# espnet/espnet

Measured on NVIDIA B200. Metric: utterances/sec (RTF) Conformer-large ASR inference at 1/2/4/8 B200 vs CPU ref, higher is better.
Workload: dtype f32

## Files before the change

espnet_b200/csrc/gemm.cu:

```cuda
#include <cuda.h>
#include <limits.h>
#include <stdio.h>
#include <stdlib.h>

#include "common.cuh"
#include "gemm.h"
#include "tc_common.cuh"

namespace {

using namespace espb::tc;

constexpr int BM = 128;
constexpr int BK = 32;
constexpr int A_TILE_BYTES = BM * 128;
constexpr int NUM_THREADS = 192;

struct EpiArgs {
  float* C; long long c_plane, ldc; int split_out;
  const float* bias; const float* R; long long ldr; float alpha; int act;
};

__device__ __forceinline__ float epi_value(const EpiArgs& e, float acc, long long row, int col) {
  float v = acc;
// ... 3 lines not shown
  if (e.R) v += e.R[row * e.ldr + col];
  return v;
}

__device__ __forceinline__ void epi_store_chunk32(const EpiArgs& e, float (&v)[32], int row, bool row_ok, int col0, int N, bool vec_ok, bool r_vec_ok) {
  float* crow = e.C + (long long)row * e.ldc;
  if (!row_ok || col0 >= N) return;
  if (vec_ok && col0 + 32 <= N) {
    float rres[32];
    if (e.R && r_vec_ok) {
      const float4* rp4 = reinterpret_cast<const float4*>(e.R + (long long)row * e.ldr + col0);
#pragma unroll
      for (int j = 0; j < 8; ++j) { const float4 t = rp4[j]; rres[4 * j] = t.x; rres[4 * j + 1] = t.y; rres[4 * j + 2] = t.z; rres[4 * j + 3] = t.w; }
    } else {
#pragma unroll
      for (int j = 0; j < 32; ++j) rres[j] = e.R ? e.R[(long long)row * e.ldr + col0 + j] : 0.f;
    }
#pragma unroll
    for (int j = 0; j < 32; ++j) {
      float x = v[j];
      if (e.bias) x += __ldg(e.bias + col0 + j);
      x = espb::apply_act_acc(x, e.act);
      v[j] = fmaf(e.alpha, x, rres[j]);
    }
#pragma unroll
    for (int j = 0; j < 32; j += 4) {
      float4 o, l;
      const float t0 = v[j], t1 = v[j + 1], t2 = v[j + 2], t3 = v[j + 3];
      if (e.split_out) {
        o.x = espb::tf32_hi(t0); o.y = espb::tf32_hi(t1); o.z = espb::tf32_hi(t2); o.w = espb::tf32_hi(t3);
        l.x = espb::tf32_lo(t0, o.x); l.y = espb::tf32_lo(t1, o.y); l.z = espb::tf32_lo(t2, o.z); l.w = espb::tf32_lo(t3, o.w);
        *reinterpret_cast<float4*>(crow + col0 + j) = o;
        *reinterpret_cast<float4*>(crow + e.c_plane + col0 + j) = l;
      } else {
        o.x = t0; o.y = t1; o.z = t2; o.w = t3;
        *reinterpret_cast<float4*>(crow + col0 + j) = o;
      }
    }
  } else {
#pragma unroll
    for (int j = 0; j < 32; ++j) {
      const int col = col0 + j;
      if (col < N) {
        const float t = epi_value(e, v[j], row, col);
        if (e.split_out) {
          const float h = espb::tf32_hi(t);
          crow[col] = h; crow[e.c_plane + col] = espb::tf32_lo(t, h);
        } else {
          crow[col] = t;
        }
      }
    }
  }
}

template <int BN, int STAGES>
__global__ void __launch_bounds__(NUM_THREADS, 1)
gemm_tf32x3_kernel(const __grid_constant__ CUtensorMap tmA, const __grid_constant__ CUtensorMap tmB, EspbGemmDesc p, int bxm, int bym, int axm, int aym) {
  constexpr int B_TILE_BYTES = BN * 128;
  constexpr int STAGE_BYTES = 2 * A_TILE_BYTES + 2 * B_TILE_BYTES;
  extern __shared__ uint8_t smem_raw[];
  const uint32_t smem_base = (smem_u32(smem_raw) + 1023u) & ~1023u;
  const uint32_t bar_base = smem_base + STAGES * STAGE_BYTES;
  const uint32_t full_bar = bar_base, empty_bar = bar_base + 8 * STAGES, tmem_full_bar = bar_base + 16 * STAGES;
  uint32_t* tmem_ptr_smem = reinterpret_cast<uint32_t*>(smem_raw + (bar_base - smem_u32(smem_raw)) + 16 * STAGES + 8);

  const int warp = threadIdx.x >> 5, lane = threadIdx.x & 31;
  const int m0 = blockIdx.x * BM, n0 = blockIdx.y * BN;
  const int bx = blockIdx.z % p.nbx, by = blockIdx.z / p.nbx;
  const int num_kb = (p.K + BK - 1) / BK;
  if (p.band_t > 0 && ((n0 + BN - 1 < p.band_t - 1 - (m0 + BM - 1)) || (n0 > 2 * p.band_t - 2 - m0))) {
    espb::pdl_wait();
    return;
  }

  if (warp == 0 && lane == 0) {
    for (int s = 0; s < STAGES; ++s) { mbar_init(full_bar + 8 * s, 1); mbar_init(empty_bar + 8 * s, 1); }
    mbar_init(tmem_full_bar, 1);
    asm volatile("fence.mbarrier_init.release.cluster;" ::: "memory");
    asm volatile("prefetch.tensormap [%0];" ::"l"(&tmA) : "memory");
    asm volatile("prefetch.tensormap [%0];" ::"l"(&tmB) : "memory");
  }
  if (warp == 1) {
    asm volatile("tcgen05.alloc.cta_group::1.sync.aligned.shared::cta.b32 [%0], %1;" ::"r"(smem_u32(tmem_ptr_smem)), "r"((uint32_t)BN) : "memory");
    asm volatile("tcgen05.relinquish_alloc_permit.cta_group::1.sync.aligned;" ::: "memory");
  }
  tcgen05_fence_before();
  __syncthreads();
  tcgen05_fence_after();
  const uint32_t tmem_base = *tmem_ptr_smem;
  espb::pdl_trigger();
  espb::pdl_wait();

  if (warp == 0) {
    if (elect_one_sync()) {
      const int cblk = (p.a_mode == 1) ? p.cv_cin / BK : 0;
      for (int kb = 0; kb < num_kb; ++kb) {
        const int s = kb % STAGES;
        const uint32_t ph = (kb / STAGES) & 1;
        mbar_wait(empty_bar + 8 * s, ph ^ 1);
        const uint32_t fb = full_bar + 8 * s;
        mbar_expect_tx(fb, STAGE_BYTES);
        const uint32_t sa = smem_base + s * STAGE_BYTES;
        if (p.a_mode == 0) {
          const int ko = (p.kob > 0) ? kb / p.kob : 0;
          const int ki = (p.kob > 0) ? kb % p.kob : kb;
// ... 48 lines not shown
    const bool r_vec_ok = p.R && ((p.ldr & 3) == 0) && ((((long long)by * p.sr_y + (long long)bx * p.sr_x) & 3) == 0) &&
                          ((reinterpret_cast<uintptr_t>(p.R) & 15) == 0);
#pragma unroll 1
    for (int c = 0; c < BN / 32; ++c) {
      float v[32];
      __syncwarp();
      tmem_ld32(tmem_base + ((uint32_t)(q * 32) << 16) + (uint32_t)(c * 32), v);
      epi_store_chunk32(e, v, row, row_ok, n0 + c * 32, p.N, vec_ok, r_vec_ok);
    }
  }
  tcgen05_fence_before();
  __syncthreads();
  if (warp == 1) {
    asm volatile("tcgen05.dealloc.cta_group::1.sync.aligned.b32 %0, %1;" ::"r"(tmem_base), "r"((uint32_t)BN) : "memory");
  }
}

template <int BN, int STAGES, int MC>
__global__ void __cluster_dims__(1, MC, 1) __launch_bounds__(NUM_THREADS, 1)
gemm_tf32x3_mc_kernel(const __grid_constant__ CUtensorMap tmA, const __grid_constant__ CUtensorMap tmB, EspbGemmDesc p, int bxm, int bym, int axm, int aym) {
  constexpr int B_TILE_BYTES = BN * 128;
  constexpr int STAGE_BYTES = 2 * A_TILE_BYTES + 2 * B_TILE_BYTES;
  extern __shared__ uint8_t smem_raw[];
  const uint32_t smem_base = (smem_u32(smem_raw) + 1023u) & ~1023u;
  const uint32_t bar_base = smem_base + STAGES * STAGE_BYTES;
  const uint32_t full_bar = bar_base, empty_bar = bar_base + 8 * STAGES, tmem_full_bar = bar_base + 16 * STAGES;
  uint32_t* tmem_ptr_smem = reinterpret_cast<uint32_t*>(smem_raw + (bar_base - smem_u32(smem_raw)) + 16 * STAGES + 8);

  const int warp = threadIdx.x >> 5, lane = threadIdx.x & 31;
  const int m0 = blockIdx.x * BM, n0 = blockIdx.y * BN;
  const int bx = blockIdx.z % p.nbx, by = blockIdx.z / p.nbx;
  const int num_kb = (p.K + BK - 1) / BK;
  const uint32_t rank = cluster_ctarank_v();
  constexpr uint16_t MASK = (uint16_t)((1u << MC) - 1);
  constexpr int SLICE_ROWS = BM / MC, SLICE_BYTES = SLICE_ROWS * 128;

  if (warp == 0 && lane == 0) {
    for (int s = 0; s < STAGES; ++s) { mbar_init(full_bar + 8 * s, 1); mbar_init(empty_bar + 8 * s, MC); }
    mbar_init(tmem_full_bar, 1);
    asm volatile("fence.mbarrier_init.release.cluster;" ::: "memory");
    asm volatile("prefetch.tensormap [%0];" ::"l"(&tmA) : "memory");
    asm volatile("prefetch.tensormap [%0];" ::"l"(&tmB) : "memory");
  }
  if (warp == 1) {
    asm volatile("tcgen05.alloc.cta_group::1.sync.aligned.shared::cta.b32 [%0], %1;" ::"r"(smem_u32(tmem_ptr_smem)), "r"((uint32_t)BN) : "memory");
    asm volatile("tcgen05.relinquish_alloc_permit.cta_group::1.sync.aligned;" ::: "memory");
  }
  tcgen05_fence_before();
  __syncthreads();
  cluster_sync_all_v();
  tcgen05_fence_after();
  const uint32_t tmem_base = *tmem_ptr_smem;
  espb::pdl_trigger();
  espb::pdl_wait();

  if (warp == 0) {
    if (elect_one_sync()) {
      for (int kb = 0; kb < num_kb; ++kb) {
        const int s = kb % STAGES;
        const uint32_t ph = (kb / STAGES) & 1;
        mbar_wait(empty_bar + 8 * s, ph ^ 1);
        const uint32_t fb = full_bar + 8 * s;
        mbar_expect_tx(fb, STAGE_BYTES);
        const uint32_t sa = smem_base + s * STAGE_BYTES;
        {
          const int ko = (p.kob > 0) ? kb / p.kob : 0;
          const int ki = (p.kob > 0) ? kb % p.kob : kb;
          const int mrow = m0 + (int)rank * SLICE_ROWS;
          tma_load_5d_mc(sa + rank * SLICE_BYTES, &tmA, fb, ki * BK, mrow, bx * axm + ko, by * aym, 0, MASK);
          tma_load_5d_mc(sa + A_TILE_BYTES + rank * SLICE_BYTES, &tmA, fb, ki * BK, mrow, bx * axm + ko, by * aym, 1, MASK);
        }
        tma_load_5d(sa + 2 * A_TILE_BYTES, &tmB, fb, kb * BK, n0, bx * bxm, by * bym, 0);
        tma_load_5d(sa + 2 * A_TILE_BYTES + B_TILE_BYTES, &tmB, fb, kb * BK, n0, bx * bxm, by * bym, 1);
      }
    }
  } else if (warp == 1) {
    if (elect_one_sync()) {
      const uint32_t idesc = (1u << 4) | (2u << 7) | (2u << 10) | ((uint32_t)(BN >> 3) << 17) | ((uint32_t)(BM >> 4) << 24);
      for (int kb = 0; kb < num_kb; ++kb) {
        const int s = kb % STAGES;
        const uint32_t ph = (kb / STAGES) & 1;
        mbar_wait(full_bar + 8 * s, ph);
        tcgen05_fence_after();
        const uint32_t sa = smem_base + s * STAGE_BYTES;
#pragma unroll
        for (int k = 0; k < BK / 8; ++k) {
          const uint64_t a_hi = umma_desc(sa + k * 32), a_lo = umma_desc(sa + A_TILE_BYTES + k * 32);
          const uint64_t b_hi = umma_desc(sa + 2 * A_TILE_BYTES + k * 32);
          const uint64_t b_lo = umma_desc(sa + 2 * A_TILE_BYTES + B_TILE_BYTES + k * 32);
          mma_tf32(tmem_base, a_lo, b_hi, idesc, (kb | k) != 0);
          mma_tf32(tmem_base, a_hi, b_lo, idesc, 1);
          mma_tf32(tmem_base, a_hi, b_hi, idesc, 1);
        }
        tcgen05_commit_mc(empty_bar + 8 * s, MASK);
      }
      tcgen05_commit(tmem_full_bar);
    }
  } else {
    const int q = warp & 3;
    mbar_wait(tmem_full_bar, 0);
    tcgen05_fence_after();
    const int row = m0 + q * 32 + lane;
    const bool row_ok = row < p.M;
    EpiArgs e;
    const long long coff = (long long)by * p.sc_y + (long long)bx * p.sc_x;
    e.C = p.C + coff; e.c_plane = p.c_plane; e.ldc = p.ldc; e.split_out = p.split_out;
    e.bias = p.bias ? p.bias + (long long)bx * p.sbias_x : nullptr; e.R = p.R ? p.R + (long long)by * p.sr_y + (long long)bx * p.sr_x : nullptr;
    e.ldr = p.ldr; e.alpha = p.alpha; e.act = p.act;
    const bool vec_ok = ((p.ldc & 3) == 0) && ((coff & 3) == 0) && ((p.c_plane & 3) == 0) &&
                        ((reinterpret_cast<uintptr_t>(p.C) & 15) == 0);
    const bool r_vec_ok = p.R && ((p.ldr & 3) == 0) && ((((long long)by * p.sr_y + (long long)bx * p.sr_x) & 3) == 0) &&
                          ((reinterpret_cast<uintptr_t>(p.R) & 15) == 0);
#pragma unroll 1
    for (int c = 0; c < BN / 32; ++c) {
      float v[32];
      __syncwarp();
      tmem_ld32(tmem_base + ((uint32_t)(q * 32) << 16) + (uint32_t)(c * 32), v);
      epi_store_chunk32(e, v, row, row_ok, n0 + c * 32, p.N, vec_ok, r_vec_ok);
    }
  }
  tcgen05_fence_before();
  __syncthreads();
  cluster_sync_all_v();
  if (warp == 1) {
    asm volatile("tcgen05.dealloc.cta_group::1.sync.aligned.b32 %0, %1;" ::"r"(tmem_base), "r"((uint32_t)BN) : "memory");
  }
}

template <int BN, int STAGES, int SK>
__global__ void __cluster_dims__(1, 1, SK) __launch_bounds__(NUM_THREADS, 1)
gemm_tf32x3_sk_kernel(const __grid_constant__ CUtensorMap tmA, const __grid_constant__ CUtensorMap tmB, EspbGemmDesc p) {
  constexpr int B_TILE_BYTES = BN * 128;
  constexpr int STAGE_BYTES = 2 * A_TILE_BYTES + 2 * B_TILE_BYTES;
  constexpr int NCHUNK = BN / 32;
  static_assert(STAGES * STAGE_BYTES >= BN * BM * 4, "partial-tile staging must fit in the pipeline buffers");
  extern __shared__ uint8_t smem_raw[];
  const uint32_t smem_base = (smem_u32(smem_raw) + 1023u) & ~1023u;
  const uint32_t bar_base = smem_base + STAGES * STAGE_BYTES;
  const uint32_t full_bar = bar_base, empty_bar = bar_base + 8 * STAGES, tmem_full_bar = bar_base + 16 * STAGES;
  uint32_t* tmem_ptr_smem = reinterpret_cast<uint32_t*>(smem_raw + (bar_base - smem_u32(smem_raw)) + 16 * STAGES + 8);

  const int warp = threadIdx.x >> 5, lane = threadIdx.x & 31;
  const int m0 = blockIdx.x * BM, n0 = blockIdx.y * BN;
  const uint32_t rank = cluster_ctarank_v();
  const int num_kb_all = (p.K + BK - 1) / BK;
  const int kb_per = (num_kb_all + SK - 1) / SK;
  const int kb0 = (int)rank * kb_per;
  const int nkb = min(num_kb_all, kb0 + kb_per) - kb0;

  if (warp == 0 && lane == 0) {
    for (int s = 0; s < STAGES; ++s) { mbar_init(full_bar + 8 * s, 1); mbar_init(empty_bar + 8 * s, 1); }
    mbar_init(tmem_full_bar, 1);
    asm volatile("fence.mbarrier_init.release.cluster;" ::: "memory");
    asm volatile("prefetch.tensormap [%0];" ::"l"(&tmA) : "memory");
    asm volatile("prefetch.tensormap [%0];" ::"l"(&tmB) : "memory");
  }
  if (warp == 1) {
    asm volatile("tcgen05.alloc.cta_group::1.sync.aligned.shared::cta.b32 [%0], %1;" ::"r"(smem_u32(tmem_ptr_smem)), "r"((uint32_t)BN) : "memory");
    asm volatile("tcgen05.relinquish_alloc_permit.cta_group::1.sync.aligned;" ::: "memory");
  }
  tcgen05_fence_before();
  __syncthreads();
  tcgen05_fence_after();
  const uint32_t tmem_base = *tmem_ptr_smem;
  espb::pdl_trigger();
  espb::pdl_wait();
  const int q = warp & 3;
  const uint32_t stg_lane = smem_base + (uint32_t)(q * 32 + lane) * 16u;

  if (warp == 0) {
    if (elect_one_sync()) {
      for (int i = 0; i < nkb; ++i) {
        const int s = i % STAGES;
        const uint32_t ph = (i / STAGES) & 1;
        mbar_wait(empty_bar + 8 * s, ph ^ 1);
        const uint32_t fb = full_bar + 8 * s;
        mbar_expect_tx(fb, STAGE_BYTES);
        const uint32_t sa = smem_base + s * STAGE_BYTES;
        const int k0 = (kb0 + i) * BK;
        tma_load_5d(sa, &tmA, fb, k0, m0, 0, 0, 0);
        tma_load_5d(sa + A_TILE_BYTES, &tmA, fb, k0, m0, 0, 0, 1);
        tma_load_5d(sa + 2 * A_TILE_BYTES, &tmB, fb, k0, n0, 0, 0, 0);
        tma_load_5d(sa + 2 * A_TILE_BYTES + B_TILE_BYTES, &tmB, fb, k0, n0, 0, 0, 1);
      }
    }
  } else if (warp == 1) {
    if (elect_one_sync()) {
      const uint32_t idesc = (1u << 4) | (2u << 7) | (2u << 10) | ((uint32_t)(BN >> 3) << 17) | ((uint32_t)(BM >> 4) << 24);
      for (int i = 0; i < nkb; ++i) {
        const int s = i % STAGES;
        const uint32_t ph = (i / STAGES) & 1;
        mbar_wait(full_bar + 8 * s, ph);
        tcgen05_fence_after();
        const uint32_t sa = smem_base + s * STAGE_BYTES;
#pragma unroll
        for (int k = 0; k < BK / 8; ++k) {
          const uint64_t a_hi = umma_desc(sa + k * 32), a_lo = umma_desc(sa + A_TILE_BYTES + k * 32);
          const uint64_t b_hi = umma_desc(sa + 2 * A_TILE_BYTES + k * 32);
          const uint64_t b_lo = umma_desc(sa + 2 * A_TILE_BYTES + B_TILE_BYTES + k * 32);
          mma_tf32(tmem_base, a_lo, b_hi, idesc, (i | k) != 0);
          mma_tf32(tmem_base, a_hi, b_lo, idesc, 1);
          mma_tf32(tmem_base, a_hi, b_hi, idesc, 1);
        }
        tcgen05_commit(empty_bar + 8 * s);
      }
      tcgen05_commit(tmem_full_bar);
    }
  } else {
    mbar_wait(tmem_full_bar, 0);
    tcgen05_fence_after();
#pragma unroll 1
    for (int c = 0; c < NCHUNK; ++c) {
      if ((uint32_t)(c % SK) == rank) continue;
      float v[32];
      __syncwarp();
      tmem_ld32(tmem_base + ((uint32_t)(q * 32) << 16) + (uint32_t)(c * 32), v);
#pragma unroll
      for (int j4 = 0; j4 < 8; ++j4) {
        const uint32_t a = stg_lane + (uint32_t)((c * 8 + j4) * BM) * 16u;
        asm volatile("st.shared.v4.f32 [%0], {%1, %2, %3, %4};" ::"r"(a), "f"(v[4 * j4]), "f"(v[4 * j4 + 1]), "f"(v[4 * j4 + 2]), "f"(v[4 * j4 + 3])
                     : "memory");
      }
    }
  }
  __syncwarp();
  cluster_sync_all_v();

  if (warp >= 2) {
    const int row = m0 + q * 32 + lane;
    const bool row_ok = row < p.M;
    EpiArgs e;
    e.C = p.C; e.c_plane = p.c_plane; e.ldc = p.ldc; e.split_out = p.split_out;
    e.bias = p.bias; e.R = p.R; e.ldr = p.ldr; e.alpha = p.alpha; e.act = p.act;
    const bool vec_ok = ((p.ldc & 3) == 0) && ((p.c_plane & 3) == 0) && ((reinterpret_cast<uintptr_t>(p.C) & 15) == 0);
    const bool r_vec_ok = p.R && ((p.ldr & 3) == 0) && ((reinterpret_cast<uintptr_t>(p.R) & 15) == 0);
#pragma unroll 1
// ... 664 lines not shown
```

espnet_b200/csrc/gemm.h:

```cpp
#pragma once
#include <cuda_runtime.h>

struct EspbGemmDesc {
  int M, N, K;
  int nbx, nby;
  int a_mode;
  int kob;
  const float* A; long long a_plane, lda, sa_x, sa_y;
  const float* B; long long b_plane, ldb, sb_x, sb_y;
  float* C; long long c_plane, ldc, sc_x, sc_y;
  int split_out;
  const float* bias;
  long long sbias_x;
  const float* R; long long ldr, sr_x, sr_y;
  float alpha;
  int act;
  int cv_t1h, cv_f1h, cv_cin;
  int band_t;
};

int espb_gemm_tc_launch(const EspbGemmDesc& d, cudaStream_t stream, int version);
int espb_gemm_simt_launch(const EspbGemmDesc& d, cudaStream_t stream);
```

espnet_b200/csrc/search_ops.cu:

```cuda
#include <stdlib.h>

#include "common.cuh"

namespace {

constexpr float LOGZERO = -10000000000.0f;
using espb::logaddexp;

__device__ __forceinline__ void store_split(float* p, long long plane, float v) {
  float h = espb::tf32_hi(v);
  p[0] = h;
  p[plane] = espb::tf32_lo(v, h);
}

__global__ void dec_embed_kernel(const int* __restrict__ last_tok, const float* __restrict__ emb, const float* __restrict__ pe, int pos,
                                 const int* __restrict__ step_ptr, int D, float scale, float* __restrict__ x) {
  espb::pdl_trigger();
  espb::pdl_wait();
  if (step_ptr) pos += *step_ptr;
  const int s = blockIdx.x;
  const float* e = emb + (long long)last_tok[s] * D;
  const float* p = pe + (long long)pos * D;
  for (int c = threadIdx.x; c < D; c += blockDim.x) x[(long long)s * D + c] = e[c] * scale + p[c];
}
// ... 411 lines not shown
      __syncthreads();
    }
    const float* tile = ring + (i % S) * TILE_F;
    {
      const int tb = (i - nt) * TR, rows = min(TR, T - tb);
      if (warp * 8 < rows) {
        const int t0 = tb + warp * 8 + t4, t1 = t0 + 4;
        uint32_t ah[4], al[4];
        split_tf32(t0 < T ? sc[sa * Tmax + t0] : 0.f, ah[0], al[0]);
        split_tf32(t0 < T ? sc[sb * Tmax + t0] : 0.f, ah[1], al[1]);
        split_tf32(t1 < T ? sc[sa * Tmax + t1] : 0.f, ah[2], al[2]);
        split_tf32(t1 < T ? sc[sb * Tmax + t1] : 0.f, ah[3], al[3]);
#pragma unroll
        for (int n8 = 0; n8 < 8; ++n8) {
          uint32_t bh[2], bl[2];
          split_tf32(tile[(warp * 8 + t4) * VST + n8 * 8 + g], bh[0], bl[0]);
          split_tf32(tile[(warp * 8 + t4 + 4) * VST + n8 * 8 + g], bh[1], bl[1]);
          mma3_tf32(acc[n8], ah, al, bh, bl);
        }
      }
    }
  }
  cp_async_wait<0>();
  __syncthreads();
  float* red = ring;
  static_assert(S * TILE_F >= 8 * 16 * DK, "reduction scratch must fit in the ring");
#pragma unroll
  for (int n8 = 0; n8 < 8; ++n8) {
    float* r0p = red + ((long long)warp * 16 + g) * DK + n8 * 8 + 2 * t4;
    float* r1p = red + ((long long)warp * 16 + g + 8) * DK + n8 * 8 + 2 * t4;
    r0p[0] = acc[n8][0]; r0p[1] = acc[n8][1];
    r1p[0] = acc[n8][2]; r1p[1] = acc[n8][3];
  }
  __syncthreads();
  for (int i = threadIdx.x; i < W * DK; i += blockDim.x) {
    const int w = i / DK, d = i % DK;
    float a = 0.f;
#pragma unroll
    for (int ww = 0; ww < 8; ++ww) a += red[((long long)ww * 16 + w) * DK + d];
    store_split(ctx + ((long long)(u * Wall + w0 + w)) * D + h * DK + d, ctx_plane, a);
  }
}

#ifndef ESPB_SRC_ATTN_NW_DEFAULT
#define ESPB_SRC_ATTN_NW_DEFAULT 4
#endif
template <int S, int NW>
__global__ void __launch_bounds__(NW * 32, 16 / NW) dec_src_attn_flash_kernel(const float* __restrict__ q, const float* __restrict__ kmem, const float* __restrict__ vmem,
                                                                    int Tmax, const int* __restrict__ lens, int W, int D, int H,
                                                                    float* __restrict__ ctx, long long ctx_plane, int w0, int Wall) {
  constexpr int DK = 64, QST = 68, ST = 68, TR = 8 * NW, TILE_F = TR * ST, STAGE_F = 2 * TILE_F;
  extern __shared__ float sm[];
  espb::pdl_trigger();
  espb::pdl_wait();
  const int u = blockIdx.x / H, h = blockIdx.x % H;
  const int T = lens[u];
  float* qlo = sm;
  float* ring = qlo + 16 * QST;
  const int warp = threadIdx.x >> 5, lane = threadIdx.x & 31;
  const int g = lane >> 2, t4 = lane & 3;
  const float4* kb = reinterpret_cast<const float4*>(kmem + ((long long)(u * H + h) * Tmax) * DK);
  const float4* vb = reinterpret_cast<const float4*>(vmem + ((long long)(u * H + h) * Tmax) * DK);
  const int nt = (T + TR - 1) / TR;
  auto issue = [&](int i) {
    if (i < nt) {
      const int tb = i * TR;
      float* dst = ring + (i % S) * STAGE_F;
#pragma unroll
      for (int j = threadIdx.x; j < 2 * TR * 16; j += NW * 32) {
        const int isv = j / (TR * 16), rr = (j >> 4) % TR, cc = j & 15;
        const bool ok = tb + rr < T;
        cp_async16_zfill(dst + isv * TILE_F + rr * ST + cc * 4, (isv ? vb : kb) + (ok ? (long long)(tb + rr) * 16 + cc : 0), ok ? 16 : 0);
      }
    }
    cp_async_commit();
  };
#pragma unroll
  for (int i = 0; i < S - 1; ++i) issue(i);
  uint32_t qh[8][4];
  {
    const float* qg = q + ((long long)(u * Wall + w0)) * D + h * DK;
#pragma unroll
    for (int ks = 0; ks < 8; ++ks) {
#pragma unroll
      for (int e = 0; e < 4; ++e) {
        const int row = g + (e & 1) * 8, col = ks * 8 + t4 + (e >> 1) * 4;
        const float x = (row < W) ? __ldg(qg + (long long)row * D + col) : 0.f;
        uint32_t lo;
        split_tf32(x, qh[ks][e], lo);
        if (warp == 0) qlo[row * QST + col] = __uint_as_float(lo);
      }
    }
  }
  const float inv_rs = 0.125f;
  float m0 = -INFINITY, m1 = -INFINITY, l0 = 0.f, l1 = 0.f;
  float acc[8][4];
#pragma unroll
  for (int n8 = 0; n8 < 8; ++n8) { acc[n8][0] = 0.f; acc[n8][1] = 0.f; acc[n8][2] = 0.f; acc[n8][3] = 0.f; }
  const int f0 = warp * 8;

  for (int i = 0; i < nt; ++i) {
    cp_async_wait<S - 2>();
    __syncthreads();
    issue(i + S - 1);
    const int tb = i * TR;
    if (tb + f0 >= T) continue;
    const float* kt = ring + (i % S) * STAGE_F;
    const float* vt = kt + TILE_F;
    float c[4] = {0.f, 0.f, 0.f, 0.f}, c1[4] = {0.f, 0.f, 0.f, 0.f}, c2[4] = {0.f, 0.f, 0.f, 0.f};
    const float* kr = kt + (f0 + g) * ST + t4;
#pragma unroll
    for (int ks = 0; ks < 8; ++ks) {
      uint32_t bh[2], bl[2], al[4];
      split_tf32(kr[ks * 8], bh[0], bl[0]);
      split_tf32(kr[ks * 8 + 4], bh[1], bl[1]);
      al[0] = __float_as_uint(qlo[g * QST + ks * 8 + t4]); al[1] = __float_as_uint(qlo[(g + 8) * QST + ks * 8 + t4]);
      al[2] = __float_as_uint(qlo[g * QST + ks * 8 + t4 + 4]); al[3] = __float_as_uint(qlo[(g + 8) * QST + ks * 8 + t4 + 4]);
      mma_m16n8k8_tf32(c1, al, bh);
      mma_m16n8k8_tf32(c2, qh[ks], bl);
      mma_m16n8k8_tf32(c, qh[ks], bh);
    }
    const int fa = tb + f0 + 2 * t4;
#pragma unroll
    for (int e = 0; e < 4; ++e) c[e] = (c[e] + (c1[e] + c2[e])) * inv_rs;
    if (fa >= T) { c[0] = -INFINITY; c[2] = -INFINITY; }
    if (fa + 1 >= T) { c[1] = -INFINITY; c[3] = -INFINITY; }
    float x0 = fmaxf(c[0], c[1]), x1 = fmaxf(c[2], c[3]);
    x0 = fmaxf(x0, __shfl_xor_sync(0xffffffffu, x0, 1)); x1 = fmaxf(x1, __shfl_xor_sync(0xffffffffu, x1, 1));
    x0 = fmaxf(x0, __shfl_xor_sync(0xffffffffu, x0, 2)); x1 = fmaxf(x1, __shfl_xor_sync(0xffffffffu, x1, 2));
    const float n0 = fmaxf(m0, x0), n1 = fmaxf(m1, x1);
    const float a0 = expf(m0 - n0), a1 = expf(m1 - n1);
// ... 701 lines not shown
```

espnet_b200/csrc/tc_common.cuh:

```cuda
#pragma once
#include <cuda.h>
#include <cuda_runtime.h>
#include <stdint.h>

namespace espb {
namespace tc {

__device__ __forceinline__ uint32_t smem_u32(const void* p) { return (uint32_t)__cvta_generic_to_shared(p); }

__device__ __forceinline__ void mbar_init(uint32_t bar, uint32_t count) {
  asm volatile("mbarrier.init.shared::cta.b64 [%0], %1;" ::"r"(bar), "r"(count) : "memory");
}
__device__ __forceinline__ void mbar_expect_tx(uint32_t bar, uint32_t bytes) {
  asm volatile("mbarrier.arrive.expect_tx.shared::cta.b64 _, [%0], %1;" ::"r"(bar), "r"(bytes) : "memory");
}
__device__ __forceinline__ void mbar_wait(uint32_t bar, uint32_t parity) {
  uint32_t done = 0;
  for (int spin = 0; ; ++spin) {
    asm volatile(
        "{\n\t.reg .pred p;\n\t"
        "mbarrier.try_wait.parity.shared::cta.b64 p, [%1], %2, %3;\n\t"
        "selp.u32 %0, 1, 0, p;\n\t}"
        : "=r"(done)
        : "r"(bar), "r"(parity), "r"(0x989680u)
        : "memory");
    if (done) break;
    if (spin > (1 << 22)) __trap();
  }
}
__device__ __forceinline__ void mbar_wait_spin(uint32_t bar, uint32_t parity) {
  uint32_t done = 0;
  for (uint32_t spin = 0; ; ++spin) {
    asm volatile(
        "{\n\t.reg .pred p;\n\t"
        "mbarrier.try_wait.parity.shared::cta.b64 p, [%1], %2;\n\t"
        "selp.u32 %0, 1, 0, p;\n\t}"
        : "=r"(done)
        : "r"(bar), "r"(parity)
        : "memory");
    if (done) break;
    if (spin > (1u << 26)) __trap();
  }
}
__device__ __forceinline__ void tma_load_5d(uint32_t dst, const CUtensorMap* map, uint32_t bar, int c0, int c1, int c2,
                                            int c3, int c4) {
  asm volatile(
      "cp.async.bulk.tensor.5d.shared::cluster.global.mbarrier::complete_tx::bytes [%0], [%1, {%3, %4, %5, %6, %7}], [%2];"
      ::"r"(dst), "l"(map), "r"(bar), "r"(c0), "r"(c1), "r"(c2), "r"(c3), "r"(c4)
      : "memory");
}
__device__ __forceinline__ void tcgen05_commit(uint32_t bar) {
  asm volatile("tcgen05.commit.cta_group::1.mbarrier::arrive::one.shared::cluster.b64 [%0];" ::"r"(bar) : "memory");
}
__device__ __forceinline__ void tcgen05_fence_after() { asm volatile("tcgen05.fence::after_thread_sync;" ::: "memory"); }
__device__ __forceinline__ void tcgen05_fence_before() { asm volatile("tcgen05.fence::before_thread_sync;" ::: "memory"); }

__device__ __forceinline__ void mma_tf32(uint32_t d_tmem, uint64_t adesc, uint64_t bdesc, uint32_t idesc, uint32_t accum) {
  asm volatile(
      "{\n\t.reg .pred p;\n\t"
      "setp.ne.b32 p, %4, 0;\n\t"
      "tcgen05.mma.cta_group::1.kind::tf32 [%0], %1, %2, %3, p;\n\t}"
      ::"r"(d_tmem), "l"(adesc), "l"(bdesc), "r"(idesc), "r"(accum)
      : "memory");
}

__device__ __forceinline__ uint64_t umma_desc(uint32_t smem_addr) {
  uint32_t lo = ((smem_addr >> 4) & 0x3FFFu) | (1u << 16);
  uint32_t hi = (1024u >> 4) | (1u << 14) | (2u << 29);
  return (uint64_t)lo | ((uint64_t)hi << 32);
}

__device__ __forceinline__ void tmem_ld32(uint32_t taddr, float* v) {
  uint32_t* r = reinterpret_cast<uint32_t*>(v);
  asm volatile(
      "tcgen05.ld.sync.aligned.32x32b.x32.b32 "
      "{%0, %1, %2, %3, %4, %5, %6, %7, %8, %9, %10, %11, %12, %13, %14, %15, "
      "%16, %17, %18, %19, %20, %21, %22, %23, %24, %25, %26, %27, %28, %29, %30, %31}, [%32];"
      : "=r"(r[0]), "=r"(r[1]), "=r"(r[2]), "=r"(r[3]), "=r"(r[4]), "=r"(r[5]), "=r"(r[6]), "=r"(r[7]), "=r"(r[8]),
        "=r"(r[9]), "=r"(r[10]), "=r"(r[11]), "=r"(r[12]), "=r"(r[13]), "=r"(r[14]), "=r"(r[15]), "=r"(r[16]),
        "=r"(r[17]), "=r"(r[18]), "=r"(r[19]), "=r"(r[20]), "=r"(r[21]), "=r"(r[22]), "=r"(r[23]), "=r"(r[24]),
        "=r"(r[25]), "=r"(r[26]), "=r"(r[27]), "=r"(r[28]), "=r"(r[29]), "=r"(r[30]), "=r"(r[31])
      : "r"(taddr)
      : "memory");
  asm volatile("tcgen05.wait::ld.sync.aligned;" ::: "memory");
}

__device__ __forceinline__ void tmem_ld16(uint32_t taddr, float* v) {
  uint32_t* r = reinterpret_cast<uint32_t*>(v);
  asm volatile(
      "tcgen05.ld.sync.aligned.32x32b.x16.b32 {%0, %1, %2, %3, %4, %5, %6, %7, %8, %9, %10, %11, %12, %13, %14, %15}, [%16];"
      : "=r"(r[0]), "=r"(r[1]), "=r"(r[2]), "=r"(r[3]), "=r"(r[4]), "=r"(r[5]), "=r"(r[6]), "=r"(r[7]), "=r"(r[8]),
        "=r"(r[9]), "=r"(r[10]), "=r"(r[11]), "=r"(r[12]), "=r"(r[13]), "=r"(r[14]), "=r"(r[15])
      : "r"(taddr)
      : "memory");
  asm volatile("tcgen05.wait::ld.sync.aligned;" ::: "memory");
}

__device__ __forceinline__ uint32_t cluster_ctarank() {
  uint32_t r;
  asm volatile("mov.u32 %0, %%cluster_ctarank;" : "=r"(r));
  return r;
}
__device__ __forceinline__ void cluster_sync_all() {
// ... 123 lines not shown
```

espnet_b200/decoder.py:

```python
import math
from typing import List

import torch

from . import ops
from .lib import call, ptr
from .ops import ACT_RELU, _count, layernorm, linear, new_split, split_from

LN_EPS = 1e-12


class _MHA(torch.nn.Module):
    def __init__(self, n_feat):
        super().__init__()
        self.linear_q = torch.nn.Linear(n_feat, n_feat)
        self.linear_k = torch.nn.Linear(n_feat, n_feat)
        self.linear_v = torch.nn.Linear(n_feat, n_feat)
        self.linear_out = torch.nn.Linear(n_feat, n_feat)


class _FFN(torch.nn.Module):
    def __init__(self, d, units):
        super().__init__()
        self.w_1 = torch.nn.Linear(d, units)
# ... 92 lines not shown
        return None if state is None else state[i]

    def final_score(self, state) -> float:
        return 0.0

    def _iface_memory(self, x, n, need_len):
        key = (x.data_ptr(), tuple(x.shape), tuple(x.stride()), x._version)
        c = getattr(self, "_iface", None)
        if c is None or c["key"] != key:
            T = x.shape[0]
            self.ws_tag = "iface"
            c = self._iface = dict(key=key, x_ref=x, enc_split=split_from(x.contiguous().float()),
                                   lens32=torch.tensor([T], dtype=torch.int32, device=x.device), T=T, st=None)
        st = c["st"]
        if st is None or st["n"] != n or st["max_len"] < need_len:
            cap = max(32, 1 << (need_len - 1).bit_length())
            self.ws_tag = "iface"
            c["st"] = st = self.init_memory(c["enc_split"], 1, c["T"], c["lens32"], n, cap)
        return st

    @torch.no_grad()
    def batch_score(self, ys: torch.Tensor, states, xs: torch.Tensor):
        n, ln = ys.shape
        pos = ln - 1
        st = self._iface_memory(xs[0], n, ln)
        self.ws_tag = "iface"
        L, D = self.num_blocks, self.d
        kc, vc = st["kc"], st["vc"]
        if pos > 0:
            kc[:, :pos] = torch.stack([s[0] for s in states], dim=2)
            vc[:, :pos] = torch.stack([s[1] for s in states], dim=2)
        anc = self._buf("iface_anc", (n, st["max_len"] + 1), dtype=torch.int32)
        anc.copy_(torch.arange(n, dtype=torch.int32, device=anc.device).view(n, 1).expand_as(anc))
        logp = self.step(st, pos, ys[:, -1].to(torch.int32).contiguous(), anc, n, None)
        new_states = [(kc[:, :ln, b].clone(), vc[:, :ln, b].clone()) for b in range(n)]
        return logp.clone(), new_states

    @torch.no_grad()
    def score(self, ys: torch.Tensor, state, x: torch.Tensor):
        logp, states = self.batch_score(ys.unsqueeze(0), [state], x.unsqueeze(0))
        return logp[0], states[0]

    @torch.no_grad()
    def init_memory(self, enc_split, U, Tmax, lens32, n_slots, max_len):
        pk = self._packed or self._pack()
        L, D, H = self.num_blocks, self.d, self.heads
        dk = D // H
        kvmem = self._buf("kvmem", (L, 2, U, H, Tmax, dk), zero=True)
        for l in range(L):
            for j in range(2):
                ops.gemm(Tmax, dk, D, enc_split, U * Tmax * D, D, pk["kv_w"], L * 2 * D * D, D, kvmem, dk, bias=pk["kv_b"],
                         nbx=H, nby=U, sa=(0, Tmax * D), sb=(dk * D, 0), sc=(Tmax * dk, H * Tmax * dk), b_off=(l * 2 + j) * D * D,
                         c_off=(l * 2 + j) * U * H * Tmax * dk, sbias_x=dk, bias_off=(l * 2 + j) * D)
        st = dict(kvmem=kvmem, U=U, Tmax=Tmax, lens32=lens32, n=n_slots, max_len=max_len,
                  kc=self._buf("kc", (L, max_len, n_slots, D)), vc=self._buf("vc", (L, max_len, n_slots, D)),
                  pe=self._pe(max_len))
        return st

    def _pe(self, length):
        key = ("pe", length)
        if key not in self._ws:
            self._ws[key] = pos_enc_table(length, self.d).to(self.after_norm.weight.device)
        return self._ws[key]

    @torch.no_grad()
    def step(self, st, pos, last_tok, anc, W, step_ptr=None):
        pk = self._packed
        n, D, H, L, Uu = st["n"], self.d, self.heads, self.num_blocks, self.units
        x = self._buf("x", (n, D))
        xn = self._buf("xn", (2, n, D))
        qkv = self._buf("qkv", (n, 3 * D))
        ctx = self._buf("ctx", (2, n, D))
        q = self._buf("q", (n, D))
        h = self._buf("h", (2, n, Uu))
        call("espb_dec_embed_f32", ptr(last_tok), ptr(pk["emb"]), ptr(st["pe"]), pos, ptr(step_ptr), n, D, math.sqrt(D), ptr(x))
        _count()
        for li, w in enumerate(pk["layers"]):
            layernorm(x, *w["n1"], LN_EPS, out_split=xn)
            linear(xn, w["qkv_w"], qkv, bias=w["qkv_b"])
            call("espb_dec_self_attn_f32", ptr(qkv), ptr(st["kc"][li]), ptr(st["vc"][li]), ptr(anc), anc.shape[1], n, D, H, pos,
                 ptr(step_ptr), st["max_len"], ptr(ctx), n * D)
            _count()
            linear(ctx, w["so_w"], x, bias=w["so_b"], residual=x)
            layernorm(x, *w["n2"], LN_EPS, out_split=xn)
            linear(xn, w["cq_w"], q, bias=w["cq_b"])
            call("espb_dec_src_attn_f32", ptr(q), ptr(st["kvmem"][li, 0]), ptr(st["kvmem"][li, 1]), st["U"], st["Tmax"],
                 ptr(st["lens32"]), W, D, H, ptr(ctx), n * D)
            _count()
            linear(ctx, w["co_w"], x, bias=w["co_b"], residual=x)
            layernorm(x, *w["n3"], LN_EPS, out_split=xn)
            linear(xn, w["w1"], h, bias=w["b1"], act=ACT_RELU, split_out=True)
            linear(h, w["w2"], x, bias=w["b2"], residual=x)
        layernorm(x, *pk["an"], LN_EPS, out_split=xn)
        logp = self._buf("logp", (n, self.odim))
        linear(xn, pk["out_w"], logp, bias=pk["out_b"])
        ops.log_softmax_rows_(logp)
        return logp
```

espnet_b200/lib.py:

```python
import ctypes
import os
from ctypes import POINTER, Structure, c_float, c_int, c_longlong, c_void_p

import torch

_HERE = os.path.dirname(os.path.abspath(__file__))
LIB_PATH = os.path.join(_HERE, "libespnet_b200.so")

_lib = None


class GemmDesc(Structure):

    _fields_ = [
        ("M", c_int), ("N", c_int), ("K", c_int), ("nbx", c_int), ("nby", c_int), ("a_mode", c_int), ("kob", c_int),
        ("A", c_void_p), ("a_plane", c_longlong), ("lda", c_longlong), ("sa_x", c_longlong), ("sa_y", c_longlong),
        ("B", c_void_p), ("b_plane", c_longlong), ("ldb", c_longlong), ("sb_x", c_longlong), ("sb_y", c_longlong),
        ("C", c_void_p), ("c_plane", c_longlong), ("ldc", c_longlong), ("sc_x", c_longlong), ("sc_y", c_longlong),
        ("split_out", c_int), ("bias", c_void_p), ("sbias_x", c_longlong),
        ("R", c_void_p), ("ldr", c_longlong), ("sr_x", c_longlong), ("sr_y", c_longlong),
        ("alpha", c_float), ("act", c_int), ("cv_t1h", c_int), ("cv_f1h", c_int), ("cv_cin", c_int), ("band_t", c_int),
    ]


P, I, L, F = c_void_p, c_int, c_longlong, c_float

_SIGS = {
    "espb_gemm_f32": [POINTER(GemmDesc), I, P],
    "espb_stft_logmel_f32": [P, P, I, I, I, P, P, P, P, P, P, P, I, I, P, I, P, P],
    "espb_utt_mvn_from_partial_f32": [P, P, I, I, I, I, P, P],
    "espb_utt_mvn_f32": [P, P, I, I, I, P, P],
    "espb_global_mvn_f32": [P, P, I, I, I, P, P, I, I, P],
    "espb_layernorm_f32": [P, L, I, P, P, F, P, P, L, P],
    "espb_split_tf32_f32": [P, L, P, L, P],
    "espb_conv1_relu_f32": [P, I, I, I, P, P, I, P, I, I, I, I, P],
    "espb_qu_qv_f32": [P, L, L, I, P, P, P, P, L, P],
    "espb_v_transpose_f32": [P, L, I, I, I, I, P, P, L, I, P],
    "espb_relpos_softmax_f32": [P, P, I, I, I, I, I, P, F, P, L, P],
    "espb_masked_softmax_f32": [P, I, I, I, I, P, F, P, L, P],
    "espb_flash_attn_f32": [P, L, L, L, P, L, L, L, P, L, I, P, I, P, I, I, I, I, P, L, L, P],
    "espb_glu_dwconv_bn_swish_f32": [P, I, I, I, P, P, P, I, P, P, P, L, P],
    "espb_zero_pad_rows_f32": [P, I, I, I, P, L, I, P],
    "espb_cbe_build_chunks_f32": [P, I, I, I, I, I, I, P, I, I, F, P, P, P, P],
    "espb_cbe_ctx_propagate_f32": [P, I, I, I, I, P, P, I, I, P],
    "espb_zero_rows_f32": [P, L, L, L, I, L, I, P],
    "espb_gather_rows_f32": [P, I, L, P, I, I, P, P],
    "espb_log_softmax_rows_f32": [P, L, L, I, P],
    "espb_argmax_rows_f32": [P, L, L, I, P, P],
    "espb_ctc_collapse_i32": [P, I, I, P, I, P, P, P],
    "espb_dec_embed_f32": [P, P, P, I, P, I, I, F, P, P],
    "espb_dec_self_attn_f32": [P, P, P, P, I, I, I, I, I, P, I, P, L, P],
    "espb_dec_src_attn_f32": [P, P, P, I, I, P, I, I, I, P, L, P],
    "espb_rows_topk_f32": [P, L, L, I, F, I, P, P, P],
    "espb_ctc_init_state_f32": [P, I, I, I, P, I, I, P, P, P],
    "espb_ctc_extend_state_f32": [P, I, I, I, I, P, I, P, P],
    "espb_ctc_score_cands_f32": [P, I, I, I, P, I, I, I, P, P, P, I, P, P, I, P, P, P, I, P],
    "espb_ctc_score_dense_f32": [P, I, I, I, P, I, I, I, P, P, P, I, P, P],
    "espb_beam_select": [P] * 18 + [I] + [P, P, P] + [I, I, I, I, I, P, P, P, I, F, F, F, I, P, P, P, P, P, I, I, P],
    "espb_anc_update_i32": [P, P, I, P, I, P, I, P],
    "espb_step_inc_i32": [P, P],
    "espb_gather_rows_split_f32": [P, P, I, I, P, L, P],
    "espb_relu_posenc_f32": [P, I, I, P, I, P, F, P],
    "espb_axpby_f32": [P, F, P, F, P, L, P],
    "espb_track_scores_f32": [P, P, P, P, P, I, P, P, P, P, P, P, I, P, I, P],
    "espb_ctc_advance_f32": [P, I, I, I, P, I, I, I, P, P, P, P, P, I, P, P, P, I, P],
    "espb_transpose_tv_f32": [P, I, I, I, P, P],
    "espb_count_active_i32": [P, I, P, P],
}

ABI_VERSION = 7
EXPORTED_SYMBOLS = sorted(list(_SIGS) + ["espb_last_error", "espb_abi_version", "espb_device_sm", "espb_frontend_blocks"])


class LibraryMissing(RuntimeError):
# ... 62 lines not shown
```

espnet_b200/ops.py:

```python
import os

import torch

from . import lib
from .lib import GemmDesc, call, ptr

ACT_NONE, ACT_RELU, ACT_SWISH = 0, 1, 2

_GEMM_MODE = os.environ.get("ESPNET_B200_GEMM", "tc2")
launch_counter = [0]
gemm_profile = None


def set_gemm_mode(mode):
    global _GEMM_MODE
    assert mode in ("tc", "tc2", "simt")
    _GEMM_MODE = mode


def gemm_mode():
    return _GEMM_MODE


def _count(n=1):
    launch_counter[0] += n


def new_split(*shape, device="cuda"):
    return torch.empty((2,) + tuple(shape), dtype=torch.float32, device=device)


def split_from(x):
    x = x.contiguous()
    out = new_split(*x.shape, device=x.device)
    call("espb_split_tf32_f32", ptr(x), x.numel(), ptr(out), x.numel())
    _count()
    return out


def gemm(M, N, K, A, a_plane, lda, B, b_plane, ldb, C, ldc, *, c_plane=0, split_out=False, bias=None, R=None, ldr=0,
         alpha=1.0, act=ACT_NONE, nbx=1, nby=1, sa=(0, 0), sb=(0, 0), sc=(0, 0), sr=(0, 0), kob=0, a_mode=0, conv=(0, 0, 0),
         a_off=0, b_off=0, c_off=0, r_off=0, sbias_x=0, bias_off=0, band_t=0, force=None):
    d = GemmDesc()
    d.M, d.N, d.K, d.nbx, d.nby, d.a_mode, d.kob = M, N, K, nbx, nby, a_mode, kob
    d.A = A.data_ptr() + 4 * a_off
    d.a_plane, d.lda, d.sa_x, d.sa_y = a_plane, lda, sa[0], sa[1]
    d.B = B.data_ptr() + 4 * b_off
    d.b_plane, d.ldb, d.sb_x, d.sb_y = b_plane, ldb, sb[0], sb[1]
    d.C = C.data_ptr() + 4 * c_off
    d.c_plane, d.ldc, d.sc_x, d.sc_y = c_plane, ldc, sc[0], sc[1]
    d.split_out = 1 if split_out else 0
    d.bias = (bias.data_ptr() + 4 * bias_off) if bias is not None else None
    d.sbias_x = sbias_x
    d.R = (R.data_ptr() + 4 * r_off) if R is not None else None
    d.ldr, d.sr_x, d.sr_y = ldr, sr[0], sr[1]
    d.alpha, d.act = float(alpha), act
    d.cv_t1h, d.cv_f1h, d.cv_cin = conv
    d.band_t = band_t
    mode = force or _GEMM_MODE
    use_tc = {"tc": 1, "tc2": 2}.get(mode, 0)
    if use_tc:
        al = [lda, ldb, a_plane, b_plane, sa[0], sa[1], sb[0], sb[1], a_off, b_off]
        if any(v % 4 for v in al):
            use_tc = 0
        if a_mode == 1 and conv[2] % 32:
            use_tc = 0
        if a_mode == 0 and kob > 0 and K % (kob * 32):
            use_tc = 0
    if lib.profile is not None:
        lib.profile_tag[0] = f"{'tc' + str(use_tc) if use_tc else 'simt'} M{M} N{N} K{K} x{nbx * nby}" + (" conv" if a_mode else "")
    prof = gemm_profile if use_tc else None
    if prof is not None:
        e0, e1 = torch.cuda.Event(enable_timing=True), torch.cuda.Event(enable_timing=True)
        e0.record()
    call("espb_gemm_f32", d, use_tc)
    if prof is not None:
        e1.record()
        n_alg = band_t if band_t > 0 else N
        prof.append((2.0 * M * n_alg * K * nbx * nby, e0, e1, use_tc == 2 and M * nbx * nby > 1024))
    _count()
    return bool(use_tc)


def linear(x_split, w_split, out, *, bias=None, act=ACT_NONE, residual=None, alpha=1.0, split_out=False, force=None):
    M, K = x_split.shape[1], x_split.shape[2]
    N = w_split.shape[1]
    assert w_split.shape[2] == K
    return gemm(M, N, K, x_split, M * K, K, w_split, N * K, K, out, N, c_plane=M * N, split_out=split_out, bias=bias,
                R=residual, ldr=N, alpha=alpha, act=act, force=force)


_ATTN_MODE = os.environ.get("ESPB_ATTN", "fused")


def set_attn_mode(mode):
    global _ATTN_MODE
    assert mode in ("fused", "materialized")
    _ATTN_MODE = mode


def attn_mode():
    return _ATTN_MODE


def use_flash_attn(dk):
    return _ATTN_MODE == "fused" and dk == 64 and _GEMM_MODE != "simt"


def flash_attn(q_split, q_off, ldq, k_split, k_off, ldk, vt, Tp, bd, Rp, lens32, B, H, T, dk, out_split):
    call("espb_flash_attn_f32", ptr(q_split), q_off, q_split[0].numel(), ldq, ptr(k_split), k_off, k_split[0].numel(), ldk, ptr(vt),
         vt[0].numel(), Tp, ptr(bd), Rp, ptr(lens32), B, H, T, dk, ptr(out_split), out_split[0].numel(), H * dk)
# ... 24 lines not shown
```

include/espnet_b200.h:

```cpp
#ifndef ESPNET_B200_H
#define ESPNET_B200_H

#include <cuda_runtime.h>

#ifdef __cplusplus
extern "C" {
#endif

#define ESPB_ACT_NONE 0
#define ESPB_ACT_RELU 1
#define ESPB_ACT_SWISH 2

const char* espb_last_error(void);
int espb_abi_version(void);
int espb_device_sm(int* major, int* minor);

typedef struct EspbGemmDesc {
  int M, N, K;
  int nbx, nby;
  int a_mode;
  int kob;
  const float* A; long long a_plane, lda, sa_x, sa_y;
  const float* B; long long b_plane, ldb, sb_x, sb_y;
  float* C; long long c_plane, ldc, sc_x, sc_y;
  int split_out;
  const float* bias; long long sbias_x;
  const float* R; long long ldr, sr_x, sr_y;
  float alpha;
  int act;
  int cv_t1h, cv_f1h, cv_cin;
  int band_t;
} EspbGemmDesc;
int espb_gemm_f32(const EspbGemmDesc* d, int use_tc, cudaStream_t stream);

int espb_frontend_blocks(int Tf_max);
int espb_stft_logmel_f32(const float* wave, const long long* wave_lens, int B, int Lmax, int hop, const float* window, const float* tw512,
                         const float* tw256t, const int* mel_start, const int* mel_count, const int* mel_offset, const float* mel_weight,
                         int mel_nnz, int n_mels, float* out, int Tf_max, float* partial, cudaStream_t stream);
int espb_utt_mvn_from_partial_f32(float* feats, const long long* wave_lens, int B, int Tf_max, int n_mels, int hop, const float* partial,
                                  cudaStream_t stream);
int espb_utt_mvn_f32(float* feats, const long long* feat_lens, int B, int Tf_max, int n_mels, float* partial_ws, cudaStream_t stream);
int espb_global_mvn_f32(float* feats, const long long* feat_lens, int B, int Tmax, int D, const float* mean, const float* stdv, int norm_means,
                        int norm_vars, cudaStream_t stream);

int espb_layernorm_f32(const float* x, long long rows, int D, const float* gamma, const float* beta, float eps, float* out_plain,
                       float* out_split, long long split_plane, cudaStream_t stream);
int espb_split_tf32_f32(const float* x, long long n, float* out, long long plane, cudaStream_t stream);
int espb_conv1_relu_f32(const float* feats, int B, int Tf_max, int F, const float* w, const float* bias, int C, float* out, int T1, int F1,
                        int T1h, int F1h, cudaStream_t stream);
int espb_qu_qv_f32(const float* qkv, long long qkv_plane, long long M, int D, const float* pos_u, const float* pos_v, float* qu, float* qv,
                   long long out_plane, cudaStream_t stream);
int espb_v_transpose_f32(const float* qkv, long long qkv_plane, int B, int Tmax, int D, int H, const int* lens, float* vt,
                         long long vt_plane, int Tp, cudaStream_t stream);
int espb_relpos_softmax_f32(const float* ac, const float* bd, int B, int H, int T, int Tp, int Rp, const int* lens, float sqrt_dk,
                            float* probs, long long probs_plane, cudaStream_t stream);
int espb_masked_softmax_f32(const float* scores, int B, int H, int T, int Tp, const int* lens, float sqrt_dk, float* probs, long long probs_plane,
                            cudaStream_t stream);
int espb_flash_attn_f32(const float* q, long long q_off, long long q_plane, long long ldq, const float* k, long long k_off, long long k_plane,
                        long long ldk, const float* vt, long long vt_plane, int Tp, const float* bd, int Rp, const int* lens, int B, int H, int T,
                        int dk, float* out, long long out_plane, long long ldo, cudaStream_t stream);
int espb_glu_dwconv_bn_swish_f32(const float* y, int B, int Tmax, int C, const int* lens, const float* dw_w, const float* dw_b, int K,
                                 const float* bn_a, const float* bn_b, float* out, long long out_plane, cudaStream_t stream);
int espb_zero_pad_rows_f32(float* x, int B, int Tmax, int D, const int* lens, long long plane, int nplanes, cudaStream_t stream);

int espb_cbe_build_chunks_f32(const float* xs, int N, int Tt, int D, int nb, int block, int hop, const float* pe, int pos0, int ctx0, float scale,
                              const float* prev_addin, float* addin_out, float* chunks, cudaStream_t stream);
int espb_cbe_ctx_propagate_f32(float* x, int N, int nb, int S, int D, const float* past_ctx, float* next_ctx, int layer, int L,
                               cudaStream_t stream);
int espb_zero_rows_f32(float* x, long long row0, long long every, long long count, int D, long long plane, int nplanes, cudaStream_t stream);
int espb_gather_rows_f32(const float* src, int N, long long src_rows, const int* idx, int nout, int D, float* out, cudaStream_t stream);

int espb_log_softmax_rows_f32(float* x, long long rows, long long ld, int V, cudaStream_t stream);
int espb_argmax_rows_f32(const float* x, long long rows, long long ld, int V, int* out, cudaStream_t stream);
int espb_ctc_collapse_i32(const int* argmax, int B, int Tmax, const int* lens, int blank, int* out_ids, int* out_len, cudaStream_t stream);

int espb_dec_embed_f32(const int* last_tok, const float* emb, const float* pe, int pos, const int* step_ptr, int n, int D, float scale, float* x,
                       cudaStream_t stream);
int espb_dec_self_attn_f32(const float* qkv, float* kc, float* vc, const int* anc, int anc_ld, int n, int D, int H, int pos, const int* step_ptr,
                           int max_pos, float* ctx, long long ctx_plane, cudaStream_t stream);
int espb_dec_src_attn_f32(const float* q, const float* kmem, const float* vmem, int U, int Tmax, const int* lens, int W, int D, int H, float* ctx,
                          long long ctx_plane, cudaStream_t stream);

int espb_rows_topk_f32(const float* x, long long rows, long long ld, int V, float scale, int k, int* ids, float* vals, cudaStream_t stream);
int espb_ctc_init_state_f32(const float* logp, int U, int Tmax, int V, const int* lens, int blank, int W, float* r, float* s_prev,
// ... 33 lines not shown
```

Baseline: 306.9.

## Issue constant weight TMA loads before PDL wait to overlap with predecessor kernel

GEMM kernels whose B operand is marked as a constant pre-split weight now issue the first STAGES weight-tile TMA loads, plus L2 prefetches of the remaining weight tiles and the bias, before the programmatic dependent launch wait. The main producer loop then skips those B loads and their expect_tx. The flash-attention-style search kernel also moves its PDL wait after its initial prefetch issues. The aim is to hide weight-fetch latency behind the tail of the previous kernel, at the cost of relying on the weights truly being written before the launch chain, and of extra L2 prefetch traffic.

```diff
diff --git a/espnet_b200/csrc/gemm.cu b/espnet_b200/csrc/gemm.cu
--- a/espnet_b200/csrc/gemm.cu
+++ b/espnet_b200/csrc/gemm.cu
@@ -79,6 +79,24 @@
       }
     }
   }
+}
+
+template <int BN>
+__device__ __forceinline__ void issue_weights_before_wait(const CUtensorMap* tmB, uint32_t smem_base, uint32_t full_bar, uint32_t stage_bytes,
+                                                          int npre, int nkb, int kb0, int n0, int c2, int c3, const float* bias) {
+  for (int i = 0; i < npre; ++i) {
+    const uint32_t fb = full_bar + 8 * i;
+    const uint32_t sb = smem_base + i * stage_bytes + 2 * A_TILE_BYTES;
+    mbar_expect_tx(fb, stage_bytes);
+    tma_load_5d(sb, tmB, fb, (kb0 + i) * BK, n0, c2, c3, 0);
+    tma_load_5d(sb + BN * 128, tmB, fb, (kb0 + i) * BK, n0, c2, c3, 1);
+  }
+  for (int i = npre; i < nkb; ++i) {
+    tma_prefetch_l2_5d(tmB, (kb0 + i) * BK, n0, c2, c3, 0);
+    tma_prefetch_l2_5d(tmB, (kb0 + i) * BK, n0, c2, c3, 1);
+  }
+  if (bias)
+    for (int c = 0; c < BN; c += 32) asm volatile("prefetch.global.L2 [%0];" ::"l"(bias + n0 + c) : "memory");
 }
 
 template <int BN, int STAGES>
@@ -233,6 +251,13 @@
   tcgen05_fence_after();
   const uint32_t tmem_base = *tmem_ptr_smem;
   espb::pdl_trigger();
+  const int npre = p.b_const ? min(num_kb, STAGES) : 0;
+  if (warp == 0 && npre > 0) {
+    if (elect_one_sync())
+      issue_weights_before_wait<BN>(&tmB, smem_base, full_bar, STAGE_BYTES, npre, num_kb, 0, n0, bx * bxm, by * bym,
+                                    p.bias ? p.bias + (long long)bx * p.sbias_x : nullptr);
+    __syncwarp();
+  }
   espb::pdl_wait();
 
   if (warp == 0) {
@@ -242,8 +267,8 @@
         const uint32_t ph = (kb / STAGES) & 1;
         mbar_wait(empty_bar + 8 * s, ph ^ 1);
         const uint32_t fb = full_bar + 8 * s;
-        mbar_expect_tx(fb, STAGE_BYTES);
         const uint32_t sa = smem_base + s * STAGE_BYTES;
+        if (kb >= npre) mbar_expect_tx(fb, STAGE_BYTES);
         {
           const int ko = (p.kob > 0) ? kb / p.kob : 0;
           const int ki = (p.kob > 0) ? kb % p.kob : kb;
@@ -251,8 +276,10 @@
           tma_load_5d_mc(sa + rank * SLICE_BYTES, &tmA, fb, ki * BK, mrow, bx * axm + ko, by * aym, 0, MASK);
           tma_load_5d_mc(sa + A_TILE_BYTES + rank * SLICE_BYTES, &tmA, fb, ki * BK, mrow, bx * axm + ko, by * aym, 1, MASK);
         }
-        tma_load_5d(sa + 2 * A_TILE_BYTES, &tmB, fb, kb * BK, n0, bx * bxm, by * bym, 0);
-        tma_load_5d(sa + 2 * A_TILE_BYTES + B_TILE_BYTES, &tmB, fb, kb * BK, n0, bx * bxm, by * bym, 1);
+        if (kb >= npre) {
+          tma_load_5d(sa + 2 * A_TILE_BYTES, &tmB, fb, kb * BK, n0, bx * bxm, by * bym, 0);
+          tma_load_5d(sa + 2 * A_TILE_BYTES + B_TILE_BYTES, &tmB, fb, kb * BK, n0, bx * bxm, by * bym, 1);
+        }
       }
     }
   } else if (warp == 1) {
@@ -345,6 +372,11 @@
   tcgen05_fence_after();
   const uint32_t tmem_base = *tmem_ptr_smem;
   espb::pdl_trigger();
+  const int npre = p.b_const ? min(nkb, STAGES) : 0;
+  if (warp == 0 && npre > 0) {
+    if (elect_one_sync()) issue_weights_before_wait<BN>(&tmB, smem_base, full_bar, STAGE_BYTES, npre, nkb, kb0, n0, 0, 0, p.bias);
+    __syncwarp();
+  }
   espb::pdl_wait();
   const int q = warp & 3;
   const uint32_t stg_lane = smem_base + (uint32_t)(q * 32 + lane) * 16u;
@@ -356,13 +388,15 @@
         const uint32_t ph = (i / STAGES) & 1;
         mbar_wait(empty_bar + 8 * s, ph ^ 1);
         const uint32_t fb = full_bar + 8 * s;
-        mbar_expect_tx(fb, STAGE_BYTES);
         const uint32_t sa = smem_base + s * STAGE_BYTES;
         const int k0 = (kb0 + i) * BK;
+        if (i >= npre) mbar_expect_tx(fb, STAGE_BYTES);
         tma_load_5d(sa, &tmA, fb, k0, m0, 0, 0, 0);
         tma_load_5d(sa + A_TILE_BYTES, &tmA, fb, k0, m0, 0, 0, 1);
-        tma_load_5d(sa + 2 * A_TILE_BYTES, &tmB, fb, k0, n0, 0, 0, 0);
-        tma_load_5d(sa + 2 * A_TILE_BYTES + B_TILE_BYTES, &tmB, fb, k0, n0, 0, 0, 1);
+        if (i >= npre) {
+          tma_load_5d(sa + 2 * A_TILE_BYTES, &tmB, fb, k0, n0, 0, 0, 0);
+          tma_load_5d(sa + 2 * A_TILE_BYTES + B_TILE_BYTES, &tmB, fb, k0, n0, 0, 0, 1);
+        }
       }
     }
   } else if (warp == 1) {
diff --git a/espnet_b200/csrc/gemm.h b/espnet_b200/csrc/gemm.h
--- a/espnet_b200/csrc/gemm.h
+++ b/espnet_b200/csrc/gemm.h
@@ -17,6 +17,7 @@
   int act;
   int cv_t1h, cv_f1h, cv_cin;
   int band_t;
+  int b_const;
 };
 
 int espb_gemm_tc_launch(const EspbGemmDesc& d, cudaStream_t stream, int version);
diff --git a/espnet_b200/csrc/search_ops.cu b/espnet_b200/csrc/search_ops.cu
--- a/espnet_b200/csrc/search_ops.cu
+++ b/espnet_b200/csrc/search_ops.cu
@@ -487,7 +487,6 @@
   constexpr int DK = 64, QST = 68, ST = 68, TR = 8 * NW, TILE_F = TR * ST, STAGE_F = 2 * TILE_F;
   extern __shared__ float sm[];
   espb::pdl_trigger();
-  espb::pdl_wait();
   const int u = blockIdx.x / H, h = blockIdx.x % H;
   const int T = lens[u];
   float* qlo = sm;
@@ -512,6 +511,7 @@
   };
 #pragma unroll
   for (int i = 0; i < S - 1; ++i) issue(i);
+  espb::pdl_wait();
   uint32_t qh[8][4];
   {
     const float* qg = q + ((long long)(u * Wall + w0)) * D + h * DK;
diff --git a/espnet_b200/csrc/tc_common.cuh b/espnet_b200/csrc/tc_common.cuh
--- a/espnet_b200/csrc/tc_common.cuh
+++ b/espnet_b200/csrc/tc_common.cuh
@@ -49,6 +49,11 @@
       ::"r"(dst), "l"(map), "r"(bar), "r"(c0), "r"(c1), "r"(c2), "r"(c3), "r"(c4)
       : "memory");
 }
+__device__ __forceinline__ void tma_prefetch_l2_5d(const CUtensorMap* map, int c0, int c1, int c2, int c3, int c4) {
+  asm volatile("cp.async.bulk.prefetch.tensor.5d.L2.global.tile [%0, {%1, %2, %3, %4, %5}];"
+               ::"l"(map), "r"(c0), "r"(c1), "r"(c2), "r"(c3), "r"(c4)
+               : "memory");
+}
 __device__ __forceinline__ void tcgen05_commit(uint32_t bar) {
   asm volatile("tcgen05.commit.cta_group::1.mbarrier::arrive::one.shared::cluster.b64 [%0];" ::"r"(bar) : "memory");
 }
diff --git a/espnet_b200/decoder.py b/espnet_b200/decoder.py
--- a/espnet_b200/decoder.py
+++ b/espnet_b200/decoder.py
@@ -168,6 +168,7 @@
                 ops.gemm(Tmax, dk, D, enc_split, U * Tmax * D, D, pk["kv_w"], L * 2 * D * D, D, kvmem, dk, bias=pk["kv_b"],
                          nbx=H, nby=U, sa=(0, Tmax * D), sb=(dk * D, 0), sc=(Tmax * dk, H * Tmax * dk), b_off=(l * 2 + j) * D * D,
                          c_off=(l * 2 + j) * U * H * Tmax * dk, sbias_x=dk, bias_off=(l * 2 + j) * D)
+        self._buf("kv_ready", (1,)).zero_()
         st = dict(kvmem=kvmem, U=U, Tmax=Tmax, lens32=lens32, n=n_slots, max_len=max_len,
                   kc=self._buf("kc", (L, max_len, n_slots, D)), vc=self._buf("vc", (L, max_len, n_slots, D)),
                   pe=self._pe(max_len))
diff --git a/espnet_b200/lib.py b/espnet_b200/lib.py
--- a/espnet_b200/lib.py
+++ b/espnet_b200/lib.py
@@ -20,6 +20,7 @@
         ("split_out", c_int), ("bias", c_void_p), ("sbias_x", c_longlong),
         ("R", c_void_p), ("ldr", c_longlong), ("sr_x", c_longlong), ("sr_y", c_longlong),
         ("alpha", c_float), ("act", c_int), ("cv_t1h", c_int), ("cv_f1h", c_int), ("cv_cin", c_int), ("band_t", c_int),
+        ("b_const", c_int),
     ]
 
 
diff --git a/espnet_b200/ops.py b/espnet_b200/ops.py
--- a/espnet_b200/ops.py
+++ b/espnet_b200/ops.py
@@ -35,6 +35,7 @@
     out = new_split(*x.shape, device=x.device)
     call("espb_split_tf32_f32", ptr(x), x.numel(), ptr(out), x.numel())
     _count()
+    out.espb_written_before_chain = True
     return out
 
 
@@ -57,6 +58,7 @@
     d.alpha, d.act = float(alpha), act
     d.cv_t1h, d.cv_f1h, d.cv_cin = conv
     d.band_t = band_t
+    d.b_const = 1 if getattr(B, "espb_written_before_chain", False) else 0
     mode = force or _GEMM_MODE
     use_tc = {"tc": 1, "tc2": 2}.get(mode, 0)
     if use_tc:
diff --git a/include/espnet_b200.h b/include/espnet_b200.h
--- a/include/espnet_b200.h
+++ b/include/espnet_b200.h
@@ -30,6 +30,7 @@
   int act;
   int cv_t1h, cv_f1h, cv_cin;
   int band_t;
+  int b_const;
 } EspbGemmDesc;
 int espb_gemm_f32(const EspbGemmDesc* d, int use_tc, cudaStream_t stream);
 
```

Result: no change. 309.4, median of 6 (+0.8%).
